# isinaltinkaya/vcfgl

Measured on AMD Instinct MI355X. Metric: site-sample GL evals/s at depth 20, 1/2/4/8 MI355X; % HBM roofline, higher is better.
Workload: dtype f64 (f32-filtered decisions, f64 fallback)

## Files before the change

### vcfgl_amd/csrc/vgl_sample.hip

```cpp
#include <stdlib.h>
#include <type_traits>

#include "vgl_common.hip.h"

#ifndef VGL_SAMPLE_SEG_TU
__global__ __launch_bounds__(256) void k_sitebase(const VglDevParams P, const VglTilePtrs T) {
    const int ls = blockIdx.x * 256 + threadIdx.x;
    if (ls >= T.n_sites) return;
    const uint64_t h = vgl_site_hash((uint64_t)(T.site0 + ls), P.site_hash_bits);
    uint64_t xb = P.x0;
#pragma unroll 1
    for (int b = 0; b < 40; ++b)
        if ((h >> b) & 1) xb = aff(P.site_pow[b], xb);
    T.site_base[ls] = xb;
    T.site_hash[ls] = h;
    if (T.tail_base) {
        uint64_t xt = VGL_TAIL_RAND48_X0;
#pragma unroll 1
        for (int b = 0; b < 40; ++b)
            if ((h >> b) & 1) xt = aff(P.site_pow[b], xt);
        T.tail_base[ls] = xt;
    }
}

template <bool ZT>
__global__ __launch_bounds__(256) void k_depth(const VglDevParams P, const VglTilePtrs T, const int chunk) {
    const int lane = threadIdx.x & 63;
    const uint32_t N = (uint32_t)P.n_samples;
    const int64_t E = (int64_t)T.n_sites * N;
    const int64_t c0 = ((int64_t)blockIdx.x * 4 + __builtin_amdgcn_readfirstlane((int)(threadIdx.x >> 6))) * chunk;
    if (c0 >= E) return;
    const int cn = (int)((E - c0 < chunk) ? (E - c0) : chunk);
    const uint32_t ls_c0 = (uint32_t)(c0 / (int64_t)N);
    const uint32_t s_c0 = (uint32_t)(c0 - (int64_t)ls_c0 * N);
    const bool big_n = N >= (uint32_t)chunk;
    auto start_of = [&](const int i, uint32_t& s_out) -> uint64_t {
        const uint32_t t = s_c0 + (uint32_t)i;
        const uint32_t add = big_n ? (uint32_t)(t >= N) : (N == 1u ? t : __umulhi(t, P.depth_magic));
        s_out = t - add * N;
        return aff(P.depth_tab[s_out], T.site_base[ls_c0 + add]);
    };

    int i = lane, next_free = 64;
    bool busy = i < cn;
    uint32_t s_i;
    uint64_t st = start_of(busy ? i : 0, s_i);
    VglPois pp = P.pois0;
    if (P.per_sample_depth) pp = P.pois[s_i];
    while (__ballot(busy)) {
        const uint64_t st1 = lcg_next(st), st2 = lcg_next(st1);
        bool neg, reject; int result;
        poisson_attempt<ZT>(pp, st1, st2, busy, P.gamma_ln_tab, P.gamma_ln_n, P.pois_zt, neg, reject, result);
        st = neg ? st1 : st2;
        const bool done = busy && !neg && !reject;
        if (done) T.dp_pre[c0 + i] = result;
        const uint64_t dm = __ballot(done);
        const int rank = (int)__builtin_amdgcn_mbcnt_hi((uint32_t)(dm >> 32), __builtin_amdgcn_mbcnt_lo((uint32_t)dm, 0u));
        const int i_n = done ? next_free + rank : i;
        next_free += __popcll(dm);
        const bool busy_n = done ? (i_n < cn) : busy;
        uint32_t s_n;
        const uint64_t st_n = start_of(busy_n ? i_n : 0, s_n);
        if (P.per_sample_depth) { const VglPois pn = P.pois[s_n]; if (done) pp = pn; }
        st = done ? st_n : st;
        i = i_n; busy = busy_n;
    }
}

#endif

template <int EQS, bool DBG, int DM, bool PREC, int LEAN, int SEG = 0>
__device__ __forceinline__ void k_sample_body(const VglDevParams& P, const VglTilePtrs& T, const int64_t wave_index) {
    constexpr bool DEFER = (LEAN >= 2);
#ifndef VGL_POOL_GROUPS
#define VGL_POOL_GROUPS 4
#endif
#ifndef VGL_POOL_ATTEMPTS
#define VGL_POOL_ATTEMPTS 2
#endif
#ifdef VGL_POOL_F64
    constexpr bool F32 = false;
#else
#ifdef VGL_PREC_F64
    constexpr bool F32 = DEFER && !PREC;
#else
    constexpr bool F32 = DEFER;
#endif
#endif
    constexpr bool P16 = F32;
    constexpr int ISZ = P16 ? 2 : 4;
    constexpr bool SLIM = (LEAN == 1 || LEAN == 2);
    constexpr bool DUMP = (LEAN == 0);
#ifdef VGL_TEST_HOOKS
    const int dbg_redo_every = P.dbg_redo_every, dbg_qs_exact = P.dbg_qs_exact;
#else
    constexpr int dbg_redo_every = 0, dbg_qs_exact = 0;
#endif
    extern __shared__ __attribute__((aligned(16))) uint8_t lds_raw[];
    const WavePos wp = wave_pos_of(P, T, wave_index);
    if (!wp.valid) return;
    const int lane = threadIdx.x & 63;
    const int N = P.n_samples;
    const int ls = wp.ls;
    const int s = wp.chunk * 64 + lane;
    const bool active = s < N;
    const size_t ev0 = (size_t)ls * N + (size_t)wp.chunk * 64;
    size_t ev = ev0 + (active ? lane : 0);
    const size_t plane = (size_t)T.n_sites * N;

    int dp = 0, a0 = 0, a1 = 0;
    int wave_total_reads = 0;
    uint64_t ad4 = 0, adf4 = 0;
    uint32_t qs0 = 0, qs1 = 0, qs2 = 0, qs3 = 0, qq0 = 0, qq1 = 0, qq2 = 0, qq3 = 0;
    uint64_t st_hap = 0, st_base = 0, st_qs = 0;
    unsigned long long c_t0 = 0, c_pois = 0, c_owner = 0, c_pool = 0, c_flush = 0, c_iter = 0, c_items = 0, c_tmp = 0;
    unsigned long long c_ntest = 0, c_gtest = 0, c_finb = 0, c_lhave = 0, c_lfin = 0, c_lhold = 0;
    if (DBG) c_t0 = clock64();
    uint64_t err_thresh = P.err_thresh;
    const bool k_strand = SLIM ? false : (LEAN == 4 ? true : (P.sample_strand != 0));
    const bool k_qsum = SLIM ? false : (LEAN == 4 ? true : (P.need_qsum != 0));
    const int k_adj = (SLIM || LEAN == 4) ? 0 : P.adjust_qs;

    const uint64_t xb = T.site_base[ls];

    if (active) {
        const VglAffine ms = P.samp_tab[s];
        const uint64_t xe = aff(ms, xb);
        st_hap = aff(P.off[1], xe);
        st_base = aff(P.off[2], xe);
        st_qs = aff(P.off[3], xe);

        int n;
        if (DM == 1) n = T.dp_pre[ev];
        else {
            uint64_t st_depth = aff(P.off[0], xe);
            VglPois pc = P.pois0;
            if (P.per_sample_depth) pc = P.pois[s];
            if (DM == 2) {
                double t = 1.0;
                int em = -1;
                uint64_t s52 = st_depth << 4;
                uint32_t k3ff = 0x3FF00000u;
                asm volatile("" : "+v"(k3ff));
                do { ++em; s52 = lcg_next52r(s52); t *= bits_1xxx_52r(s52, k3ff) - 1.0; } while (t > pc.g);
                n = em;
            } else n = poisson_draw_fast(pc, st_depth, P.gamma_ln_tab, P.gamma_ln_n);
        }
        const uint32_t g = T.gt[ev];
        a0 = g & 0xF; a1 = (g >> 4) & 0xF;
        dp = (a0 == 0xF || a1 == 0xF) ? 0 : n;
        if (dp > P.read_cap) { atomicOr(T.errflag, VGL_DEVERR_CAPACITY); dp = P.read_cap; }
#ifdef VGL_EXP_FIXED_DP
        if (EQS != 2 && dp > 0) dp = VGL_EXP_FIXED_DP;
#endif
    }

    if (DBG) c_pois = clock64() - c_t0;
    if (DBG && P.dbg_phase == 1) return;
    if (EQS == 1) {
        uint32_t lo = 0, hi = 0;
        if (lane == 0) {
            uint64_t st_site = aff(P.off[3], aff(P.samp_tab[0], xb));
            const double pe = beta_draw(P, st_site);
            if (T.site_pick_err && wp.chunk == 0) T.site_pick_err[ls] = pe;
            const uint64_t th = (uint64_t)ceil(ldexp(pe, 48));
            lo = (uint32_t)th; hi = (uint32_t)(th >> 32);
        }
        lo = __shfl(lo, 0, 64); hi = __shfl(hi, 0, 64);
        err_thresh = ((uint64_t)hi << 32) | lo;
    }

    if (EQS != 2) {
        const int q_i = P.pre_q, aq_i = P.pre_adjq;
        const uint32_t q_gl = (uint32_t)((P.adjust_qs & 1) ? aq_i : q_i);
        const uint32_t qq = (uint32_t)((P.adjust_qs & 2) ? aq_i : q_i);
        const uint32_t q2 = (uint32_t)qs_to_qssq((int)qq);
        const bool stage = P.stage_fixed != 0;
        uint64_t st_hap16 = st_hap << 16, st_base16 = st_base << 16;
        const uint64_t err_thresh16 = sample_thresh16(err_thresh);
        uint32_t* const reads_w = (uint32_t*)T.reads;
        if (SLIM) {
            const uint32_t qrep = (q_gl << 2) * 0x01010101u;
            uint32_t* const col = reads_w + ev;
            auto emit = [&](const int trip, const uint32_t bases) { if (stage) col[(size_t)trip * plane] = staged_word_of(bases, qrep); };
#ifdef VGL_FIXED_READS_V1
            const bool narrow = false;
#else
            const bool narrow = P.read_cap <= 255;
#endif
            if (narrow) {
                if (__ballot(active && dp > 0 && a0 != a1) == 0) ad4 = sample_reads_fixed<true>(st_hap16, st_base16, a0, a1, dp, err_thresh16, emit);
                else ad4 = sample_reads_fixed<false>(st_hap16, st_base16, a0, a1, dp, err_thresh16, emit);
            } else {
                if (__ballot(active && dp > 0 && a0 != a1) == 0) ad4 = sample_reads_fixed_wide<true>(st_hap16, st_base16, a0, a1, dp, err_thresh16, emit);
                else ad4 = sample_reads_fixed_wide<false>(st_hap16, st_base16, a0, a1, dp, err_thresh16, emit);
            }
        } else
        for (int r0 = 0; r0 < dp; r0 += 4) {
            uint32_t rw = 0;
#pragma unroll
            for (int j = 0; j < 4; ++j) {
                const int r = r0 + j;
                if (r < dp) {
                    bool fwd;
                    const int r_base = sample_read_base16(st_hap16, st_base16, a0, a1, err_thresh16, k_strand, fwd);
                    rw |= ((q_gl << 2) | (uint32_t)r_base) << (8 * j);
                    if (DUMP) { if (T.reads_out && r < T.reads_out_cap) T.reads_out[(size_t)r * plane + ev] = (uint8_t)((q_i << 2) | r_base); }
                    const uint64_t one = 1ULL << (16 * r_base);
                    ad4 += one;
                    if (k_strand) { if (fwd) adf4 += one; }
                }
            }
            if (stage) reads_w[(size_t)(r0 >> 2) * plane + ev] = rw;
        }
        if (P.need_qsum) {
            qs0 = qq * (uint32_t)(ad4 & 0xFFFF); qs1 = qq * (uint32_t)((ad4 >> 16) & 0xFFFF);
            qs2 = qq * (uint32_t)((ad4 >> 32) & 0xFFFF); qs3 = qq * (uint32_t)((ad4 >> 48) & 0xFFFF);
            qq0 = q2 * (uint32_t)(ad4 & 0xFFFF); qq1 = q2 * (uint32_t)((ad4 >> 16) & 0xFFFF);
            qq2 = q2 * (uint32_t)((ad4 >> 32) & 0xFFFF); qq3 = q2 * (uint32_t)((ad4 >> 48) & 0xFFFF);
        }
    } else {
        const int cap = P.pool_cap;
        uint8_t* wl = lds_raw;
        uint64_t* l_stq = (uint64_t*)wl;
        double* l_gc = (double*)(wl + 512);
        uint32_t* l_it = (uint32_t*)(wl + 576);
        uint8_t* l_pb = wl + 576 + 4 * ((size_t)cap + 2);
        uint32_t* l_ctr = l_it + cap + 1;
        const bool qfast = (LEAN >= 3) && (P.qsum_lds != 0);
        uint32_t* l_accB = (uint32_t*)(wl + ((576 + 4 * ((size_t)cap + 2) + (size_t)cap + 7) & ~(size_t)7));
        if ((uint32_t)(uintptr_t)(__attribute__((address_space(3))) uint8_t*)lds_raw != 0u) {
            if (lane == 0) atomicOr(T.errflag, VGL_DEVERR_INTERNAL);
            return;
        }

        const int incl = (int)wave_incl_scan_u32((uint32_t)dp);
        const int offs = incl - dp;
        const int total = __builtin_amdgcn_readlane(incl, 63);
        wave_total_reads = total;
        l_stq[lane] = st_qs << 4;
        uint8_t* const l_lut = wl + ((576 + 2 * ((size_t)cap + 2) + 7) & ~(size_t)7);
        uint32_t* const l_qs = (uint32_t*)(l_lut + (P.n_qs_bins != 0 ? 256 : 0));
        double* const l_gcd = (double*)((uint8_t*)l_qs + ((LEAN >= 3 && P.qsum_lds) ? 1024 : 0));
        if (F32 && PREC) { if (lane == 0) { l_gcd[0] = P.gx.a1; l_gcd[1] = P.gx.a2; l_gcd[2] = P.gy.a1; l_gcd[3] = P.gy.a2; } }
        if (P16 && P.n_qs_bins != 0) {
#pragma unroll
            for (int j = 0; j < 4; ++j) {
                const int qv = lane * 4 + j;
                int b = 0xFF;
                for (int i = 0; i < P.n_qs_bins; ++i) if (b == 0xFF && qv >= P.qs_bins[3 * i] && qv <= P.qs_bins[3 * i + 1]) b = P.qs_bins[3 * i + 2] & 0xFF;
                l_lut[qv] = (uint8_t)b;
            }
        }
        if (P16 && LEAN >= 3) { if (P.qsum_lds) { ((uint64_t*)l_qs)[2 * lane] = 0ULL; ((uint64_t*)l_qs)[2 * lane + 1] = 0ULL; } }
        if (lane == 0) {
            if (!P16) l_it[cap] = 0u;
            if (F32) {
                float* const gf = (float*)l_gc;
                gf[0] = (float)P.gx.a1; gf[1] = (float)P.gx.a2; gf[2] = (float)((((P.gx.a2 * P.gx.a2) * 0.15) * (1.0 + 1e-5) + 1e-8) * 4294967296.0); gf[3] = (float)((P.sure_margin + 3e-7) * 4294967296.0);
                gf[4] = (float)P.gy.a1; gf[5] = (float)P.gy.a2; gf[6] = (float)((((P.gy.a2 * P.gy.a2) * 0.15) * (1.0 + 1e-5) + 1e-8) * 4294967296.0); gf[7] = (float)((P.sure_margin + 3e-7) * 4294967296.0);
            } else {
            l_gc[0] = P.gx.a1; l_gc[1] = P.gx.a2; l_gc[2] = (P.gx.a2 * P.gx.a2) * 0.15; l_gc[3] = P.sure_margin;
            l_gc[4] = P.gy.a1; l_gc[5] = P.gy.a2; l_gc[6] = (P.gy.a2 * P.gy.a2) * 0.15; l_gc[7] = P.sure_margin;
            }
        }
        int rdone = 0;
        uint32_t carry_w = 0;
        uint64_t st_hap16 = st_hap << 16, st_base16 = st_base << 16;
        const uint64_t err_thresh16 = sample_thresh16(err_thresh);
        uint8_t* reads_v = T.reads;
        uint8_t* reads_out_v = DUMP ? T.reads_out : nullptr;
        int reads_out_cap_v = (DUMP && T.reads_out) ? T.reads_out_cap : 0;
        if (!DUMP) { if constexpr (SEG != 1) asm volatile("" : "+v"(reads_v)); }
        else asm volatile("" : "+v"(reads_v), "+v"(reads_out_v), "+v"(reads_out_cap_v));

        const bool homw = __ballot(active && dp > 0 && a0 != a1) == 0;
        const int nseg = (total + cap - 1) / (cap > 0 ? cap : 1);
        const int seglen = nseg > 1 ? (total + nseg - 1) / nseg : cap;
        auto run_segment = [&](auto single_tag, const int seg0) -> bool {
            constexpr bool SINGLE = decltype(single_tag)::value;
            (void)SINGLE;
            const int segT = (total - seg0 < seglen) ? (total - seg0) : seglen;
            if (DBG) c_tmp = clock64();
            int r_end = seg0 + segT - offs; r_end = r_end > dp ? dp : r_end; r_end = r_end < rdone ? rdone : r_end;
            {
                typedef __attribute__((address_space(3))) uint32_t lds_u32o;
                typedef __attribute__((address_space(3))) uint8_t lds_u8o;
                typedef __attribute__((address_space(3))) uint16_t lds_u16o;
                const uint32_t lane4 = (uint32_t)lane << 2;
                uint32_t sv = P16 ? (((uint32_t)lane << 10) | ((uint32_t)rdone << 2)) : (((uint32_t)lane << 19) | ((uint32_t)rdone << 4));
                const uint32_t sv_end = P16 ? (((uint32_t)lane << 10) | ((uint32_t)r_end << 2)) : (((uint32_t)lane << 19) | ((uint32_t)r_end << 4));
                uint32_t ka = 576u + (uint32_t)ISZ * (uint32_t)(offs + rdone - seg0);
                uint32_t pa = 576u + 4u * ((uint32_t)cap + 2u) + (uint32_t)(offs + rdone - seg0);
                auto owner_reads = [&](auto hom_tag) {
                    constexpr bool HOMW = decltype(hom_tag)::value;
                    if constexpr (SLIM) {
                        uint32_t n1 = 0;
                        const uint32_t nrd = (sv_end > sv) ? ((sv_end - sv) >> (P16 ? 2 : 4)) : 0u;
#ifdef VGL_OWNER_READS_V2
                        uint32_t hl = (uint32_t)(st_hap16 >> 12), hh = (uint32_t)(st_hap16 >> 44), bl = (uint32_t)(st_base16 >> 12), bh = (uint32_t)(st_base16 >> 44);
                        const uint32_t t_lo = (uint32_t)(err_thresh16 >> 12), t_hi = (uint32_t)(err_thresh16 >> 44);
                        while (sv < sv_end) {
                            uint32_t rb = (uint32_t)a0;
                            if (!HOMW) {
                                lcg52_step(hl, hh, hl, hh);
                                const uint32_t h = (hh >> 19) & 1u;
                                n1 += h;
                                rb = h ? (uint32_t)a1 : (uint32_t)a0;
                            }
                            lcg52_step(bl, bh, bl, bh);
                            if (__builtin_expect((bh & 0xFFFFFu) <= t_hi, 0)) {
                                if ((bh & 0xFFFFFu) < t_hi || bl < t_lo) {
                                    const uint32_t tb = rb;
                                    do { lcg52_step(bl, bh, bl, bh); rb = (bh >> 18) & 3u; } while (rb == tb);
                                    ad4 += (1ULL << (16 * rb)) - (1ULL << (16 * tb));
                                }
                            }
                            if (P16) { *(lds_u16o*)(uintptr_t)ka = (uint16_t)(sv | rb); sv += 4u; ka += 2u; }
                            else { *(lds_u32o*)(uintptr_t)ka = sv; *(lds_u8o*)(uintptr_t)pa = (uint8_t)rb; sv += 16u; ka += 4u; pa += 1u; }
                        }
                        if constexpr (SEG != 1) {
                            st_hap16 = ((((uint64_t)(hh & 0xFFFFFu)) << 32) | hl) << 12;
                            st_base16 = ((((uint64_t)(bh & 0xFFFFFu)) << 32) | bl) << 12;
                        }
#else
                        while (sv < sv_end) {
                            uint32_t rb = (uint32_t)a0;
                            if (!HOMW) {
                                st_hap16 = lcg_next16(st_hap16);
                                const uint32_t h = (uint32_t)(st_hap16 >> 63);
                                n1 += h;
                                rb = h ? (uint32_t)a1 : (uint32_t)a0;
                            }
                            st_base16 = lcg_next16(st_base16);
                            if (st_base16 < err_thresh16) {
                                const uint32_t tb = rb;
                                do { st_base16 = lcg_next16(st_base16); rb = (uint32_t)(st_base16 >> 62); } while (rb == tb);
                                ad4 += (1ULL << (16 * rb)) - (1ULL << (16 * tb));
                            }
                            if (P16) { *(lds_u16o*)(uintptr_t)ka = (uint16_t)(sv | rb); sv += 4u; ka += 2u; }
                            else { *(lds_u32o*)(uintptr_t)ka = sv; *(lds_u8o*)(uintptr_t)pa = (uint8_t)rb; sv += 16u; ka += 4u; pa += 1u; }
                        }
#endif
                        ad4 += (((uint64_t)(nrd - n1)) << (16 * (a0 & 3))) + (((uint64_t)n1) << (16 * (a1 & 3)));
                    } else if constexpr (P16) {
                        uint32_t n1 = 0, nf = 0, nf1 = 0;
                        const uint32_t nrd = (sv_end > sv) ? ((sv_end - sv) >> 2) : 0u;
                        while (sv < sv_end) {
                            uint32_t rb = (uint32_t)a0, h = 0;
                            if (!HOMW) {
                                st_hap16 = lcg_next16(st_hap16);
                                h = (uint32_t)(st_hap16 >> 63);
                                n1 += h;
                                rb = h ? (uint32_t)a1 : (uint32_t)a0;
                            }
                            const uint32_t tb = rb;
                            st_base16 = lcg_next16(st_base16);
                            const bool err = st_base16 < err_thresh16;
                            if (err) { do { st_base16 = lcg_next16(st_base16); rb = (uint32_t)(st_base16 >> 62); } while (rb == tb); }
                            uint32_t f = 1u;
                            if (k_strand) { st_base16 = lcg_next16(st_base16); f = (uint32_t)(~st_base16 >> 63); }
                            nf += f; nf1 += f & h;
                            if (err) {
                                const uint64_t d = (1ULL << (16 * rb)) - (1ULL << (16 * tb));
                                ad4 += d;
                                if (f) adf4 += d;
                            }
                            *(lds_u16o*)(uintptr_t)ka = (uint16_t)(sv | rb); sv += 4u; ka += 2u;
                        }
                        ad4 += (((uint64_t)(nrd - n1)) << (16 * (a0 & 3))) + (((uint64_t)n1) << (16 * (a1 & 3)));
                        adf4 += (((uint64_t)(nf - nf1)) << (16 * (a0 & 3))) + (((uint64_t)nf1) << (16 * (a1 & 3)));
                    } else
                    while (sv < sv_end) {
                        bool fwd;
                        const int r_base = sample_read_base16<HOMW>(st_hap16, st_base16, a0, a1, err_thresh16, k_strand, fwd);
                        const uint64_t one = 1ULL << (16 * r_base);
                        ad4 += one;
                        if (!SLIM) { if (fwd) adf4 += one; }
                        if (P16) { *(lds_u16o*)(uintptr_t)ka = (uint16_t)(sv | (uint32_t)r_base); sv += 4u; ka += 2u; }
                        else {
                            *(lds_u32o*)(uintptr_t)ka = sv;
                            *(lds_u8o*)(uintptr_t)pa = (uint8_t)((LEAN >= 3) ? (lane4 | (uint32_t)r_base) : (uint32_t)r_base);
                            sv += 16u; ka += 4u; pa += 1u;
                        }
                    }
                };
                if (homw) owner_reads(std::true_type{}); else owner_reads(std::false_type{});
            }
            if (lane == 0) {
                if (P16) ((uint16_t*)l_it)[segT] = 0; else { l_it[segT] = 0u; *l_ctr = 128u * 4u; }
            }
            __builtin_amdgcn_fence(__ATOMIC_RELEASE, "wavefront");
            __builtin_amdgcn_wave_barrier();
            __builtin_amdgcn_fence(__ATOMIC_ACQUIRE, "wavefront");

            if (DBG) { const unsigned long long c = clock64(); c_owner += c - c_tmp; c_tmp = c; c_items += segT; }
            if (DBG && P.dbg_phase == 2) return true;
            {
                typedef __attribute__((address_space(3))) uint32_t lds_u32;
                typedef __attribute__((address_space(3))) uint16_t lds_u16;
                constexpr int NGRP = F32 ? VGL_POOL_GROUPS : 1;
                const int grpQ = (segT + NGRP - 1) / NGRP;
                const int grp = (NGRP > 1) ? (lane / (64 / NGRP)) : 0, gl = (NGRP > 1) ? (lane % (64 / NGRP)) : lane;
                const int beg = grp * grpQ;
                const int endg = (beg + grpQ < segT) ? (beg + grpQ) : segT;
                const int segT4 = (NGRP > 1 || P16) ? endg * ISZ : segT * ISZ;
                int k = (beg + gl) * ISZ, kn = (beg + gl + 64 / NGRP) * ISZ;
                bool have = k < segT4;
                bool stage1 = false;
                uint64_t st = 0; double gx = 0.0; uint32_t it_m = 0;
                uint32_t sk = 0;
                if (have) {
                    if (P16) { sk = ((const uint16_t*)l_it)[beg + gl]; st = aff52(P.qs_read_tab[(sk >> 2) & 0xFFu], l_stq[sk >> 10]); }
                    else { it_m = l_it[beg + gl]; st = aff52(P.qs_read_tab[(it_m & 0xFFFFu) >> 4], l_stq[it_m >> 19]); }
                }
                if (NGRP > 1 || P16) {
                    if (gl == 0) *(lds_u32*)(uintptr_t)(544u + 4u * (uint32_t)grp) = (uint32_t)(beg + 2 * (64 / NGRP)) * (uint32_t)ISZ;
                    __builtin_amdgcn_fence(__ATOMIC_RELEASE, "wavefront");
                    __builtin_amdgcn_wave_barrier();
                    __builtin_amdgcn_fence(__ATOMIC_ACQUIRE, "wavefront");
                }
                const bool any_changed = (P.gx.changed | P.gy.changed) != 0;
                int slow_cnt = P.slow_period, slow_cnt_n = P.slow_period_n;
                uint32_t k3ff = 0x3FF00000u;
                __attribute__((address_space(3))) uint32_t* ctr_p = (NGRP > 1 || P16) ? (__attribute__((address_space(3))) uint32_t*)(uintptr_t)(544u + 4u * (uint32_t)grp)
                                                                                : (__attribute__((address_space(3))) uint32_t*)l_ctr;
                uint32_t four_v = (uint32_t)ISZ;
                asm volatile("" : "+v"(ctr_p), "+v"(four_v));
                if constexpr (F32) {
                    typedef __attribute__((address_space(3))) float lds_f32;
                    uint32_t s_lo = (uint32_t)st, s_hi = (uint32_t)(st >> 32);
                    float gxf = 0.0f;
                    double gxd = 0.0;
                    do {
                        if (DBG) { c_iter++; c_lhave += (unsigned)__popcll(__builtin_amdgcn_ballot_w64(have)); }
                        const bool full = (--slow_cnt == 0);
                        if (full) slow_cnt = P.slow_period;
                        const bool full_n = full;
                        uint32_t goff = stage1 ? 528u : 512u;
                        asm volatile("" : "+v"(goff));
                        const lds_f32* const gc = (const lds_f32*)(uintptr_t)goff;
                        const float ga1 = gc[0], ga2 = gc[1], c015s = gc[2], sure_ms = gc[3];
                        uint32_t l1, h1, l2, h2, l3, h3;
                        lcg52_step(s_lo, s_hi, l1, h1);
                        lcg52_step(l1, h1, l2, h2);
                        lcg52_step(l2, h2, l3, h3);
                        const float ufA = pool32_u(lcg52_top32(l1, h1));
                        const float svA = pool32_sv(lcg52_top32(l2, h2));
                        const float qA = pool32_q(ufA, svA);
                        const bool q_lo = qA > VGL_P32_QLO - VGL_P32_QBAND, q_hi = qA > VGL_P32_QHI + VGL_P32_QBAND;
                        bool slow_n = false;
                        const bool n_amb = have && q_lo && !q_hi;
                        bool hold = n_amb && !full_n;
                        bool redo = false;
                        if (full_n && __builtin_amdgcn_ballot_w64(n_amb)) {
                            bool und;
                            if (DBG) c_ntest++;
                            slow_n = pool32_normal_slow(svA * __builtin_amdgcn_rcpf(ufA), ufA, qA, n_amb, und);
                            redo = und || (n_amb && dbg_redo_every && (l1 >> 8) % (uint32_t)(dbg_redo_every | (dbg_redo_every == 0)) == 0u);
                        }
                        const bool accA = !(q_lo && (q_hi || slow_n));
#if VGL_POOL_ATTEMPTS == 2
                        uint32_t l4, h4, l5, h5;
                        lcg52_step(l3, h3, l4, h4);
                        lcg52_step(l4, h4, l5, h5);
                        const float ufB = pool32_u(lcg52_top32(l3, h3));
                        const float svB = pool32_sv(lcg52_top32(l4, h4));
                        const float qB = pool32_q(ufB, svB);
                        const bool rejA = have && !hold && !accA && !redo;
                        const bool useB = rejA && !(qB > VGL_P32_QLO - VGL_P32_QBAND);
                        const bool rejB = rejA && (qB > VGL_P32_QHI + VGL_P32_QBAND);
                        const float uf = useB ? ufB : ufA, sv = useB ? svB : svA;
                        const float u2f = useB ? pool32_u(lcg52_top32(l5, h5)) : ufB;
                        const bool g_try0 = (have && accA && !hold) || useB;
#else
                        const float uf = ufA, sv = svA;
                        const float u2f = pool32_u(lcg52_top32(l3, h3));
                        const bool g_try0 = have && accA && !hold;
#endif
                        asm volatile("s_waitcnt lgkmcnt(0)" : "+v"(kn));
#ifdef VGL_POOL_CLAMP_NEXT
                        const uint32_t kc = (uint32_t)(kn < segT4 ? kn : segT * ISZ);
#else
                        const uint32_t kc = P16 ? (uint32_t)kn : (uint32_t)(kn < segT4 ? kn : segT * ISZ);
#endif
                        uint32_t rd16, ow8, skn = 0;
                        if (P16) {
                            skn = *(const lds_u16*)(uintptr_t)(576u + kc);
                            asm volatile("" : "+v"(skn));
                            rd16 = (skn << 2) & 0xFF0u;
                            ow8 = (skn >> 7) & 0x1F8u;
                        } else {
                            rd16 = *(const lds_u16*)(uintptr_t)(576u + kc);
                            ow8 = *(const lds_u16*)(uintptr_t)(578u + kc);
                            asm volatile("" : "+v"(rd16), "+v"(ow8));
                        }
                        const VglAffine tab_n = *(const VglAffine*)((const uint8_t*)P.qs_read_tab + rd16);
                        const uint64_t base_n = *(__attribute__((address_space(3))) const uint64_t*)(uintptr_t)ow8;
                        const float xn = sv * __builtin_amdgcn_rcpf(uf);
                        const float w = __builtin_fmaf(ga2, xn, 1.0f);
                        const float vv = (w * w) * w;
                        const float xsq = xn * xn;
                        const float x4 = xsq * xsq;
                        const bool sure = (0x1p32f - u2f) >= __builtin_fmaf(x4, c015s, sure_ms);
                        const bool in_range = (w >= 0.5f) && (uf >= VGL_P32_UMIN);
                        redo = redo || (g_try0 && !in_range);
                        const bool g_try = g_try0 && in_range;
                        const bool g_amb = g_try && !sure;
                        hold = hold || (g_amb && !full);
                        bool slow_g = false;
                        if (full && __builtin_amdgcn_ballot_w64(g_amb)) {
                            bool und;
                            if (DBG) c_gtest++;
                            slow_g = pool32_gamma_slow(u2f, ga2 * xn, ga1, x4, g_amb, und);
                            redo = redo || und || (g_amb && dbg_redo_every && (l3 >> 8) % (uint32_t)(dbg_redo_every | (dbg_redo_every == 0)) == 1u);
                        }
                        const bool acc_g = g_try && !(g_amb && slow_g) && !hold;
#if VGL_POOL_ATTEMPTS == 2
                        {
                            const uint32_t t_lo = useB ? l5 : l3, t_hi = useB ? h5 : h3;
                            const uint32_t r_lo = rejB ? l4 : l2, r_hi = rejB ? h4 : h2;
                            s_lo = hold ? s_lo : (g_try0 ? t_lo : r_lo);
                            s_hi = hold ? s_hi : (g_try0 ? t_hi : r_hi);
                        }
#else
                        s_lo = hold ? s_lo : (g_try0 ? l3 : l2);
                        s_hi = hold ? s_hi : (g_try0 ? h3 : h2);
#endif
                        const float val = ga1 * vv;
                        const bool fin = (acc_g && stage1) || redo;
                        const float gx_prev = gxf;
                        if constexpr (PREC) {
#ifdef VGL_EXP_NO_CHAIN
                            if (false) {
#else
                            if (acc_g) {
#endif
#if VGL_POOL_ATTEMPTS == 2
                                const uint32_t ulo = useB ? l3 : l1, uhi = useB ? h3 : h1, vlo = useB ? l4 : l2, vhi = useB ? h4 : h2;
#else
                                const uint32_t ulo = l1, uhi = h1, vlo = l2, vhi = h2;
#endif
                                const double ud = bits_1xxx_52r(((uint64_t)uhi << 32) | ulo, k3ff) - 1.0;
                                const double vd = 1.7156 * (bits_1xxx_52r(((uint64_t)vhi << 32) | vlo, k3ff) - 1.5);
                                const __attribute__((address_space(3))) double* const gd = (const __attribute__((address_space(3))) double*)(uintptr_t)((uint32_t)(uintptr_t)(__attribute__((address_space(3))) uint8_t*)l_gcd + (stage1 ? 16u : 0u));
                                const double a1d = gd[0], a2d = gd[1];
                                const double xd = div_inrange(vd, ud);
                                const double wd = 1.0 + a2d * xd;
                                const double vald = a1d * (wd * wd * wd);
                                if (stage1) {
                                    if (!redo) {
                                        const size_t ei = vgl_errp_index((int)((sk >> 2) & 0xFFu), ev0 + (sk >> 10), P.read_cap);
#ifdef VGL_EXP_NO_ERRP_STORE
                                        const double epx = div_inrange(gxd, gxd + vald); if (epx > 2.0) T.errp[ei] = epx;
#else
                                        T.errp[ei] = div_inrange(gxd, gxd + vald);
#endif
                                    }
                                } else gxd = vald;
                            }
                        }
                        gxf = (acc_g && !stage1) ? val : gxf;
                        stage1 = (stage1 != acc_g) && !redo;
                        if (DBG) {
                            const uint64_t fm = __builtin_amdgcn_ballot_w64(fin);
                            c_finb += (fm != 0); c_lfin += (unsigned)__popcll(fm); c_lhold += (unsigned)__popcll(__builtin_amdgcn_ballot_w64(hold));
                        }
                        if (fin) {
                            const float pf = gx_prev * __builtin_amdgcn_rcpf(gx_prev + val);
                            if (P16) {
                                int q_i, aq_i;
                                bool ok = qs_decide_fix(P, pf, q_i, aq_i, k_adj) && !redo;
                                if (dbg_redo_every) ok = ok && ((uint32_t)(seg0 + (k >> 1)) % (uint32_t)(dbg_redo_every | (dbg_redo_every == 0))) != 2u;
                                uint32_t qv, aqv = 0;
                                if (P.n_qs_bins != 0) {
                                    const uint32_t b = l_lut[q_i < 255 ? q_i : 255];
                                    uint32_t b2 = 0;
                                    if (!SLIM) { if (k_adj) { const int a_ = aq_i < 0 ? 0 : aq_i; b2 = l_lut[a_ < 255 ? a_ : 255]; } }
                                    const bool nobin = ok && (b == 0xFFu || b2 == 0xFFu);
                                    if (__builtin_expect(__builtin_amdgcn_ballot_w64(nobin) != 0, 0)) { if (nobin) atomicOr(T.errflag, VGL_DEVERR_QSBIN); }
                                    qv = (b == 0xFFu) ? 0u : b; aqv = (b2 == 0xFFu) ? 0u : b2;
                                } else {
                                    qv = (uint32_t)((q_i > CAP_BASEQ) ? CAP_BASEQ : q_i);
                                    if (!SLIM) aqv = (uint32_t)((aq_i > CAP_BASEQ) ? CAP_BASEQ : (aq_i < 0 ? 0 : aq_i));
                                }
                                const uint32_t q_gl = SLIM ? qv : ((k_adj & 1) ? aqv : qv), q_sum = SLIM ? 0u : ((k_adj & 2) ? aqv : qv);
                                uint32_t hi6 = ok ? ((q_gl << 2) | (q_sum << 9)) : 0x100u;
                                asm volatile("" : "+v"(hi6));
                                *(lds_u16*)(uintptr_t)(576u + (uint32_t)k) = (uint16_t)(hi6 | (sk & 3u));
                                if (!SLIM) {
                                    if (qfast && k_qsum && ok)
                                        __hip_atomic_fetch_add(l_qs + ((sk >> 10) * 4u + (sk & 3u)), q_sum + ((q_sum * q_sum) << 13), __ATOMIC_RELAXED, __HIP_MEMORY_SCOPE_WAVEFRONT);
                                }
                                sk = skn;
                            } else
                            *(lds_u32*)(uintptr_t)(576u + (uint32_t)k) = redo ? 0x7FC00000u : __float_as_uint(pf);
                            aff52_step(tab_n, (uint32_t)base_n, (uint32_t)(base_n >> 32), s_lo, s_hi);
                            k = kn;
                            asm volatile("" : "+v"(k));
                            asm volatile("ds_add_rtn_u32 %0, %1, %2" : "+v"(kn) : "v"(ctr_p), "v"(four_v) : "memory");
                        }
                        have = k < segT4;
                    } while (__builtin_amdgcn_ballot_w64(have));
                } else
                do {
                    if (DBG) c_iter++;
                    const bool full = (--slow_cnt == 0);
                    if (full) slow_cnt = P.slow_period;
                    const bool full_n = (--slow_cnt_n == 0);
                    if (full_n) slow_cnt_n = P.slow_period_n;
                    uint32_t goff = stage1 ? 32u : 0u;
                    asm volatile("" : "+v"(goff));
                    const __attribute__((address_space(3))) double* gc = (const __attribute__((address_space(3))) double*)(uintptr_t)goff + 64;
                    const double ga1 = gc[0], ga2 = gc[1], ga2sq015 = gc[2], sure_margin = gc[3];
                    uint64_t st1 = lcg_next52r(st);
                    asm volatile("" : "+v"(st1));
                    const uint64_t st2 = lcg_next52r(st1);
                    const uint64_t st3 = lcg_next52r(st2);
                    const double u = bits_1xxx_52r(st1, k3ff) - 1.0;
                    const double v = 1.7156 * (bits_1xxx_52r(st2, k3ff) - 1.5);
                    const double x = u - 0.449871;
                    const double y = fabs(v) + 0.386595;
                    const double q = (x * x) + y * (0.19600 * y - 0.25472 * x);
                    const bool q_lo = q > 0.27597, q_hi = q > 0.27846;
                    bool slow_n = false;
                    const bool n_amb = have && q_lo && !q_hi;
                    bool hold = n_amb && !full_n;
                    bool redo = false;
                    if (full_n && __builtin_amdgcn_ballot_w64(n_amb)) {
                        bool und;
                        slow_n = normal_slow_test_t<DEFER>(v, u, n_amb, und);
                        if (DEFER) redo = und || (n_amb && dbg_redo_every && ((uint32_t)(st1 >> 8) % (uint32_t)(dbg_redo_every | (dbg_redo_every == 0))) == 0u);
                    }
                    const bool acc_n = !(q_lo && (q_hi || slow_n));
                    asm volatile("s_waitcnt lgkmcnt(0)" : "+v"(kn));
                    const uint32_t kc = (uint32_t)(kn < segT4 ? kn : segT4);
                    uint32_t rd16 = *(const lds_u16*)(uintptr_t)(576u + kc);
                    uint32_t ow8 = *(const lds_u16*)(uintptr_t)(578u + kc);
                    asm volatile("" : "+v"(rd16), "+v"(ow8));
                    const uint32_t m_n = PREC ? (rd16 | (ow8 << 16)) : 0u;
                    const VglAffine tab_n = *(const VglAffine*)((const uint8_t*)P.qs_read_tab + rd16);
                    const uint64_t base_n = *(__attribute__((address_space(3))) const uint64_t*)(uintptr_t)ow8;
                    const double xn = div_inrange(v, u);
                    const double w = 1.0 + ga2 * xn;
                    const bool w_pos = w > 0.0;
                    const double vv = w * w * w;
                    const double u2 = bits_1xxx_52r(st3, k3ff) - 1.0;
                    const double xsq = xn * xn;
                    const double x4 = xsq * xsq;
                    const bool sq_fail = u2 > 1.0 - 0.0331 * x4;
                    const bool sure = (1.0 - u2 >= __builtin_fma(ga2sq015, x4, sure_margin)) && (w >= 0.5);
                    const bool g_try = have && acc_n && w_pos && !hold;
                    const bool g_amb = g_try && sq_fail && !sure;
                    hold = hold || (g_amb && !full);
                    bool slow_g = false;
                    if (full && __builtin_amdgcn_ballot_w64(g_amb)) {
                        bool und;
                        slow_g = gamma_slow_test_t<DEFER>(u2, xsq, ga1, vv, ga2 * xn, g_amb, und);
                        if (DEFER) redo = redo || und || (g_amb && dbg_redo_every && ((uint32_t)(st3 >> 8) % (uint32_t)(dbg_redo_every | (dbg_redo_every == 0))) == 1u);
                    }
                    const bool acc_g = g_try && !(g_amb && slow_g) && !hold;
                    st = hold ? st : (g_try ? st3 : st2);
                    double val = ga1 * vv;
                    if (!DEFER && __builtin_expect(any_changed, 0)) {
                        asm volatile("" ::: "memory");
                        if (acc_g && (stage1 ? P.gy.changed : P.gx.changed)) {
                            double u3;
                            do { st = lcg_next52r(st); u3 = bits_1xxx_52r(st, k3ff) - 1.0; } while (u3 == 0.0);
                            val = pow(u3, 1.0 / (stage1 ? P.gy.alpha0 : P.gx.alpha0)) * ga1 * vv;
                        }
                    }
                    const bool fin = (acc_g && stage1) || redo;
                    const uint64_t st_n = tab_n.a * base_n + tab_n.c;
                    const double gx_prev = gx;
                    gx = (acc_g && !stage1) ? val : gx;
                    stage1 = (stage1 != acc_g) && !redo;
                    if (fin) {
                        *(lds_u32*)(uintptr_t)(576u + (uint32_t)k) = __float_as_uint(qs_stage_pf(gx_prev, val));
                        if (DEFER) { if (redo) *(lds_u32*)(uintptr_t)(576u + (uint32_t)k) = 0x7FC00000u; }
                        if (PREC) {
                            const size_t ei = vgl_errp_index((int)((it_m & 0xFFFFu) >> 4), ev0 + (it_m >> 19), P.read_cap);
                            T.errp[ei] = (DEFER ? div_inrange(gx_prev, gx_prev + val) : gx_prev / (gx_prev + val));
                            it_m = m_n;
                        }
                        st = st_n;
                        k = kn;
                        asm volatile("" : "+v"(k));
                        asm volatile("ds_add_rtn_u32 %0, %1, %2" : "+v"(kn) : "v"(ctr_p), "v"(four_v) : "memory");
                    }
                    have = k < segT4;
                } while (__builtin_amdgcn_ballot_w64(have));
                asm volatile("s_waitcnt lgkmcnt(0)" : "+v"(kn) : : "memory");
            }
            __builtin_amdgcn_fence(__ATOMIC_RELEASE, "wavefront");
            __builtin_amdgcn_wave_barrier();
            __builtin_amdgcn_fence(__ATOMIC_ACQUIRE, "wavefront");

            if constexpr (SEG == 1) { uint32_t l2 = (uint32_t)lane; asm volatile("" : "+v"(l2)); ev = ev0 + (active ? (size_t)l2 : 0); }
            if (DBG) { const unsigned long long c = clock64(); c_pool += c - c_tmp; c_tmp = c; }
            if (DBG && P.dbg_phase == 3) return true;
            if (!P16 && qfast && k_qsum) {
                l_stq[lane] = 0ULL;
                ((uint64_t*)l_accB)[lane] = 0ULL;
                __builtin_amdgcn_fence(__ATOMIC_RELEASE, "wavefront");
                __builtin_amdgcn_wave_barrier();
                __builtin_amdgcn_fence(__ATOMIC_ACQUIRE, "wavefront");
            }
            const int n_pass = P16 ? 0 : ((segT + 63) >> 6);
            const int dB = (qfast && !P16) ? (n_pass | 1) : 0;
            for (int jp = 0; jp < (qfast ? dB : n_pass); ++jp) {
                const int kb = qfast ? jp : 64 * jp;
                const int kstep = qfast ? dB : 1;
                const int kk = kb + lane * kstep;
                const bool inb = kk < segT;
                const float pf = __uint_as_float(l_it[inb ? kk : cap]);
                int q_i, aq_i;
                bool ok = qs_decide_pf(P, pf, q_i, aq_i, k_adj, F32 ? VGL_P32_TF_EXTRA : 0.0f) && !dbg_qs_exact;
                if (DEFER) { if (dbg_redo_every) ok = ok && ((uint32_t)(seg0 + kk) % (uint32_t)(dbg_redo_every | (dbg_redo_every == 0))) != 2u; }
                uint64_t amb = __ballot(inb && !ok);
                if (__builtin_expect(amb != 0, 0)) {
                    while (amb) {
                        const int b = __builtin_ctzll(amb);
                        amb &= amb - 1;
                        const int Kb = seg0 + kb + b * kstep;
                        if (active && Kb >= offs && Kb < offs + dp) {
                            if (DEFER) {
                                const uint32_t part = (uint32_t)wave_index & (VGL_REDO_PARTS - 1);
                                const uint32_t idx = atomicAdd(T.redo_count + VGL_REDO_STRIDE * part, 1u);
                                if (idx < T.redo_cap) T.redo_list[(size_t)part * T.redo_cap + idx] = ((unsigned long long)ev << 10) | (unsigned long long)(Kb - offs);
                                else { const size_t bit = ev * (size_t)P.read_cap + (size_t)(Kb - offs); atomicOr(&T.redo_bits[bit >> 5], 1u << (bit & 31)); }
                            } else {
                                VglAffine jr = P.qs_read_tab[Kb - offs]; jr.c >>= 4;
                                uint64_t st_x = aff(jr, l_stq[lane] >> 4);
                                const double ep = beta_draw(P, st_x);
                                int qe, aqe;
                                errprob_raw(P, ep, qe, aqe);
                                if (aqe < 0 && (P.adjust_qs & 3)) atomicOr(T.errflag, VGL_DEVERR_ADJQ);
                                l_it[kb + b * kstep] = (uint32_t)(uint16_t)qe | ((uint32_t)(uint16_t)aqe << 16);
                            }
                        }
                    }
                    if (!DEFER) {
                        __builtin_amdgcn_fence(__ATOMIC_RELEASE, "wavefront");
                        __builtin_amdgcn_wave_barrier();
                        __builtin_amdgcn_fence(__ATOMIC_ACQUIRE, "wavefront");
                        if (inb && !ok) { const uint32_t e = l_it[kk]; q_i = (int)(int16_t)(e & 0xFFFF); aq_i = (int)(int16_t)(e >> 16); }
                    } else if (inb && !ok) { q_i = 0; aq_i = SLIM ? -1 : 0; }
                }
                qs_finish(P, q_i, aq_i, T.errflag, DEFER ? (inb && ok) : inb);
                if (SLIM) { if (inb) l_pb[kk] = (uint8_t)((q_i << 2) | l_pb[kk]); }
                else if (qfast) {
                    if (inb) {
                        const uint32_t pb = l_pb[kk];
                        const uint32_t q_s = (uint32_t)((k_adj & 1) ? aq_i : q_i);
                        l_pb[kk] = (uint8_t)((q_s << 2) | (pb & 3u));
                        if (k_qsum) {
                            uint32_t* const slot = ((pb & 2u) ? l_accB : (uint32_t*)l_stq) + ((pb >> 2) * 2u + (pb & 1u));
                            __hip_atomic_fetch_add(slot, q_s + ((q_s * q_s) << 13), __ATOMIC_RELAXED, __HIP_MEMORY_SCOPE_WAVEFRONT);
                        }
                    }
                }
                else if (inb) l_it[kk] = (uint32_t)(q_i & 0xFF) | ((uint32_t)(aq_i & 0xFF) << 8);
            }
            __builtin_amdgcn_fence(__ATOMIC_RELEASE, "wavefront");
            __builtin_amdgcn_wave_barrier();
            __builtin_amdgcn_fence(__ATOMIC_ACQUIRE, "wavefront");

            uint32_t sq0 = 0, sq1 = 0, sq2 = 0, sq3 = 0, sqq0 = 0, sqq1 = 0, sqq2 = 0, sqq3 = 0;
            if (P16) {
                const uint8_t* const it8 = (const uint8_t*)l_it;
                uint8_t* reads_f = reads_v;
                if constexpr (SEG == 1) { reads_f = T.reads; asm volatile("" : "+v"(reads_f)); }
                for (int r0 = rdone & ~3; r0 < r_end; r0 += 4) {
                    uint32_t w_lo, w_hi;
                    __builtin_memcpy(&w_lo, it8 + 2 * (offs + r0 - seg0), 4);
                    __builtin_memcpy(&w_hi, it8 + 2 * (offs + r0 - seg0) + 4, 4);
                    const uint32_t w4 = __builtin_amdgcn_perm(w_hi, w_lo, 0x06040200u);
                    const int lo = rdone > r0 ? rdone - r0 : 0, hi = r_end - r0 < 4 ? r_end - r0 : 4;
                    const uint32_t mask = (0xFFFFFFFFu << (8 * lo)) & (0xFFFFFFFFu >> (8 * (4 - hi)));
                    const uint32_t rw = (w4 & mask) | ((r0 < rdone) ? carry_w : 0u);
                    ((uint32_t*)reads_f)[(size_t)(r0 >> 2) * plane + ev] = rw;
                    carry_w = rw;
                    uint32_t und4 = __builtin_amdgcn_perm(w_hi, w_lo, 0x07050301u) & mask & 0x01010101u;
                    if (__builtin_expect(und4 != 0u, 0)) {
                        while (und4) {
                            const int j = __builtin_ctz(und4) >> 3;
                            und4 &= und4 - 1;
                            const uint32_t part = (uint32_t)wave_index & (VGL_REDO_PARTS - 1);
                            const uint32_t idx = atomicAdd(T.redo_count + VGL_REDO_STRIDE * part, 1u);
                            if (idx < T.redo_cap) T.redo_list[(size_t)part * T.redo_cap + idx] = ((unsigned long long)ev << 10) | (unsigned long long)(r0 + j);
                            else { const size_t bit = ev * (size_t)P.read_cap + (size_t)(r0 + j); atomicOr(&T.redo_bits[bit >> 5], 1u << (bit & 31)); }
                        }
                    }
                    if (!SLIM) {
                        if (k_qsum && !qfast) {
#pragma unroll
                            for (int j = 0; j < 4; ++j) {
                                const uint32_t sl = ((j < 2 ? w_lo : w_hi) >> (16 * (j & 1))) & 0xFFFFu;
                                const bool mine = (r0 + j >= rdone) && (r0 + j < r_end) && !(sl & 0x100u);
                                const uint32_t qq = mine ? ((sl >> 9) & 63u) : 0u, q2 = (uint32_t)qs_to_qssq((int)qq), rb = sl & 3u;
                                sq0 += (rb == 0) ? qq : 0u; sq1 += (rb == 1) ? qq : 0u; sq2 += (rb == 2) ? qq : 0u; sq3 += (rb == 3) ? qq : 0u;
                                sqq0 += (rb == 0) ? q2 : 0u; sqq1 += (rb == 1) ? q2 : 0u; sqq2 += (rb == 2) ? q2 : 0u; sqq3 += (rb == 3) ? q2 : 0u;
                            }
                        }
                    }
                }
            } else if (SLIM || qfast) {
                for (int r0 = rdone & ~3; r0 < r_end; r0 += 4) {
                    uint32_t w4;
                    __builtin_memcpy(&w4, l_pb + (offs + r0 - seg0), 4);
                    const int lo = rdone > r0 ? rdone - r0 : 0, hi = r_end - r0 < 4 ? r_end - r0 : 4;
                    const uint32_t mask = (0xFFFFFFFFu << (8 * lo)) & (0xFFFFFFFFu >> (8 * (4 - hi)));
                    const uint32_t rw = (w4 & mask) | ((r0 < rdone) ? carry_w : 0u);
                    ((uint32_t*)reads_v)[(size_t)(r0 >> 2) * plane + ev] = rw;
                    carry_w = rw;
                }
            } else
            for (int r0 = rdone & ~3; r0 < r_end; r0 += 4) {
                uint32_t rw = (r0 < rdone) ? carry_w : 0u;
#pragma unroll
                for (int j = 0; j < 4; ++j) {
                    const int r = r0 + j;
                    if (r >= rdone && r < r_end) {
                        const int k = offs + r - seg0;
                        const int r_base = l_pb[k] & 3;
                        const uint32_t qe = l_it[k];
                        const int q_i = (int)(qe & 0xFF);
                        const int aq_i = k_adj ? (int)((qe >> 8) & 0xFF) : -1;
                        const int q_gl = (k_adj & 1) ? aq_i : q_i;
                        rw |= (uint32_t)((q_gl << 2) | r_base) << (8 * j);
                        if (DUMP) { if (r < reads_out_cap_v) reads_out_v[(size_t)r * plane + ev] = (uint8_t)((q_i << 2) | r_base); }
                        if (k_qsum) {
                            const uint32_t qq = (uint32_t)((k_adj & 2) ? aq_i : q_i);
                            const uint32_t q2 = (uint32_t)qs_to_qssq((int)qq);
                            sq0 += (r_base == 0) ? qq : 0u; sq1 += (r_base == 1) ? qq : 0u;
                            sq2 += (r_base == 2) ? qq : 0u; sq3 += (r_base == 3) ? qq : 0u;
                            sqq0 += (r_base == 0) ? q2 : 0u; sqq1 += (r_base == 1) ? q2 : 0u;
                            sqq2 += (r_base == 2) ? q2 : 0u; sqq3 += (r_base == 3) ? q2 : 0u;
                        }
                    }
                }
                ((uint32_t*)reads_v)[(size_t)(r0 >> 2) * plane + ev] = rw;
                carry_w = rw;
            }
            rdone = r_end;
            if (!SLIM) {
                if (P16 && qfast && k_qsum) {
                    const uint64_t v01 = ((const uint64_t*)l_qs)[2 * lane], v23 = ((const uint64_t*)l_qs)[2 * lane + 1];
                    sq0 = (uint32_t)v01 & 0x1FFFu; sqq0 = (uint32_t)v01 >> 13; sq1 = (uint32_t)(v01 >> 32) & 0x1FFFu; sqq1 = (uint32_t)(v01 >> 32) >> 13;
                    sq2 = (uint32_t)v23 & 0x1FFFu; sqq2 = (uint32_t)v23 >> 13; sq3 = (uint32_t)(v23 >> 32) & 0x1FFFu; sqq3 = (uint32_t)(v23 >> 32) >> 13;
                    ((uint64_t*)l_qs)[2 * lane] = 0ULL; ((uint64_t*)l_qs)[2 * lane + 1] = 0ULL;
                } else if (qfast && k_qsum) {
                    const uint64_t v01 = l_stq[lane], v23 = ((const uint64_t*)l_accB)[lane];
                    sq0 = (uint32_t)v01 & 0x1FFFu; sqq0 = (uint32_t)v01 >> 13; sq1 = (uint32_t)(v01 >> 32) & 0x1FFFu; sqq1 = (uint32_t)(v01 >> 32) >> 13;
                    sq2 = (uint32_t)v23 & 0x1FFFu; sqq2 = (uint32_t)v23 >> 13; sq3 = (uint32_t)(v23 >> 32) & 0x1FFFu; sqq3 = (uint32_t)(v23 >> 32) >> 13;
                    if (seg0 + seglen < total) {
                        __builtin_amdgcn_fence(__ATOMIC_RELEASE, "wavefront"); __builtin_amdgcn_wave_barrier();
                        if (active) l_stq[lane] = aff(P.off[3], aff(P.samp_tab[s], xb)) << 4;
                        else l_stq[lane] = 0ULL;
                    }
                }
                if (k_qsum) {
                    if (active) {
                        uint32_t* q = T.qsum + (size_t)ls * 4 * N + s;
                        if (seg0 == 0) { q[0] = sq0; q[(size_t)N] = sq1; q[(size_t)2 * N] = sq2; q[(size_t)3 * N] = sq3; }
                        else { q[0] += sq0; q[(size_t)N] += sq1; q[(size_t)2 * N] += sq2; q[(size_t)3 * N] += sq3; }
                        if (P.need_qsumsq) {
                            uint32_t* qq = T.qsumsq + (size_t)ls * 4 * N + s;
                            if (seg0 == 0) { qq[0] = sqq0; qq[(size_t)N] = sqq1; qq[(size_t)2 * N] = sqq2; qq[(size_t)3 * N] = sqq3; }
                            else { qq[0] += sqq0; qq[(size_t)N] += sqq1; qq[(size_t)2 * N] += sqq2; qq[(size_t)3 * N] += sqq3; }
                        }
                    }
// ... 309 lines not shown
```

Measured before the change: 6.208 billion.

## Run two gamma-stage attempts per pool iteration in f32 lean kernels

Adds a HALVES path for the f32 non-precise lean variants. Each loop iteration now tries the first gamma stage and then a second, fast-path-only attempt at the next stage using fresh LCG draws, so one iteration can finish a whole beta sample instead of needing two iterations. The aim is fewer loop iterations, less lane divergence and fewer waits per completed sample. The cost is more work per iteration, wasted draws when lanes hold or finish early, and higher register pressure. The shared table prefetch is factored into a lambda used by both paths.

```diff
diff --git a/vcfgl_amd/csrc/vgl_sample.hip b/vcfgl_amd/csrc/vgl_sample.hip
--- a/vcfgl_amd/csrc/vgl_sample.hip
+++ b/vcfgl_amd/csrc/vgl_sample.hip
@@ -78,6 +78,9 @@
 #ifndef VGL_POOL_ATTEMPTS
 #define VGL_POOL_ATTEMPTS 2
 #endif
+#ifndef VGL_POOL_HALVES
+#define VGL_POOL_HALVES 3
+#endif
 #ifdef VGL_POOL_F64
     constexpr bool F32 = false;
 #else
@@ -89,6 +92,7 @@
 #endif
     constexpr bool P16 = F32;
     constexpr int ISZ = P16 ? 2 : 4;
+    constexpr bool HALVES = F32 && !PREC && ((VGL_POOL_HALVES >> (LEAN == 2 ? 0 : (LEAN == 4 ? 1 : 2))) & 1) != 0;
     constexpr bool SLIM = (LEAN == 1 || LEAN == 2);
     constexpr bool DUMP = (LEAN == 0);
 #ifdef VGL_TEST_HOOKS
@@ -441,6 +445,109 @@
                         asm volatile("" : "+v"(goff));
                         const lds_f32* const gc = (const lds_f32*)(uintptr_t)goff;
                         const float ga1 = gc[0], ga2 = gc[1], c015s = gc[2], sure_ms = gc[3];
+                        uint32_t skn = 0;
+                        VglAffine tab_n;
+                        uint64_t base_n;
+                        auto prefetch = [&]() {
+                            asm volatile("s_waitcnt lgkmcnt(0)" : "+v"(kn));
+#ifdef VGL_POOL_CLAMP_NEXT
+                            const uint32_t kc = (uint32_t)(kn < segT4 ? kn : segT * ISZ);
+#else
+                            const uint32_t kc = P16 ? (uint32_t)kn : (uint32_t)(kn < segT4 ? kn : segT * ISZ);
+#endif
+                            uint32_t rd16, ow8;
+                            if (P16) {
+                                skn = *(const lds_u16*)(uintptr_t)(576u + kc);
+                                asm volatile("" : "+v"(skn));
+                                rd16 = (skn << 2) & 0xFF0u;
+                                ow8 = (skn >> 7) & 0x1F8u;
+                            } else {
+                                rd16 = *(const lds_u16*)(uintptr_t)(576u + kc);
+                                ow8 = *(const lds_u16*)(uintptr_t)(578u + kc);
+                                asm volatile("" : "+v"(rd16), "+v"(ow8));
+                            }
+                            tab_n = *(const VglAffine*)((const uint8_t*)P.qs_read_tab + rd16);
+                            base_n = *(__attribute__((address_space(3))) const uint64_t*)(uintptr_t)ow8;
+                        };
+                        bool hold, redo, fin;
+                        float fx, fy;
+                        if constexpr (HALVES) {
+                            uint32_t l1, h1, l2, h2, l3, h3;
+                            lcg52_step(s_lo, s_hi, l1, h1);
+                            lcg52_step(l1, h1, l2, h2);
+                            lcg52_step(l2, h2, l3, h3);
+                            const float ufA = pool32_u(lcg52_top32(l1, h1));
+                            const float svA = pool32_sv(lcg52_top32(l2, h2));
+                            const float u2A = pool32_u(lcg52_top32(l3, h3));
+                            const float qA = pool32_q(ufA, svA);
+                            const bool q_lo = qA > VGL_P32_QLO - VGL_P32_QBAND, q_hi = qA > VGL_P32_QHI + VGL_P32_QBAND;
+                            const bool n_amb = have && q_lo && !q_hi;
+                            bool slow_n = false;
+                            hold = n_amb && !full;
+                            redo = false;
+                            const float xnA = svA * __builtin_amdgcn_rcpf(ufA);
+                            if (full && __builtin_amdgcn_ballot_w64(n_amb)) {
+                                bool und;
+                                if (DBG) c_ntest++;
+                                slow_n = pool32_normal_slow(xnA, ufA, qA, n_amb, und);
+                                redo = und || (n_amb && dbg_redo_every && (l1 >> 8) % (uint32_t)(dbg_redo_every | (dbg_redo_every == 0)) == 0u);
+                            }
+                            const bool g_try0 = have && !hold && !(q_lo && (q_hi || slow_n));
+                            prefetch();
+                            const float wA = __builtin_fmaf(ga2, xnA, 1.0f);
+                            const float xsqA = xnA * xnA;
+                            const float x4A = xsqA * xsqA;
+                            const bool sureA = (0x1p32f - u2A) >= __builtin_fmaf(x4A, c015s, sure_ms);
+                            const bool in_rangeA = (wA >= 0.5f) && (ufA >= VGL_P32_UMIN);
+                            redo = redo || (g_try0 && !in_rangeA);
+                            const bool g_try = g_try0 && in_rangeA;
+                            const bool g_amb = g_try && !sureA;
+                            hold = hold || (g_amb && !full);
+                            bool slow_g = false;
+                            if (full && __builtin_amdgcn_ballot_w64(g_amb)) {
+                                bool und;
+                                if (DBG) c_gtest++;
+                                slow_g = pool32_gamma_slow(u2A, ga2 * xnA, ga1, x4A, g_amb, und);
+                                redo = redo || und || (g_amb && dbg_redo_every && (l3 >> 8) % (uint32_t)(dbg_redo_every | (dbg_redo_every == 0)) == 1u);
+                            }
+                            const bool acc1 = g_try && !(g_amb && slow_g) && !hold;
+                            const float val1 = ga1 * ((wA * wA) * wA);
+                            const bool fin1 = (acc1 && stage1) || redo;
+                            s_lo = hold ? s_lo : (g_try0 ? l3 : l2);
+                            s_hi = hold ? s_hi : (g_try0 ? h3 : h2);
+                            gxf = (acc1 && !stage1) ? val1 : gxf;
+                            stage1 = (stage1 != acc1) && !redo;
+                            uint32_t goff2 = stage1 ? 528u : 512u;
+                            asm volatile("" : "+v"(goff2));
+                            const lds_f32* const gc2 = (const lds_f32*)(uintptr_t)goff2;
+                            const float gb1 = gc2[0], gb2 = gc2[1], c015s2 = gc2[2], sure_ms2 = gc2[3];
+                            uint32_t m1, n1, m2, n2, m3, n3;
+                            lcg52_step(s_lo, s_hi, m1, n1);
+                            lcg52_step(m1, n1, m2, n2);
+                            lcg52_step(m2, n2, m3, n3);
+                            const float ufB = pool32_u(lcg52_top32(m1, n1));
+                            const float svB = pool32_sv(lcg52_top32(m2, n2));
+                            const float u2B = pool32_u(lcg52_top32(m3, n3));
+                            const float qB = pool32_q(ufB, svB);
+                            const bool run2 = have && !hold && !fin1;
+                            const bool rej2 = run2 && (qB > VGL_P32_QHI + VGL_P32_QBAND);
+                            const float xnB = svB * __builtin_amdgcn_rcpf(ufB);
+                            const float wB = __builtin_fmaf(gb2, xnB, 1.0f);
+                            const float xsqB = xnB * xnB;
+                            const float x4B = xsqB * xsqB;
+                            const bool sureB = (0x1p32f - u2B) >= __builtin_fmaf(x4B, c015s2, sure_ms2);
+                            const bool in_rangeB = (wB >= 0.5f) && (ufB >= VGL_P32_UMIN);
+                            const bool acc2 = run2 && !(qB > VGL_P32_QLO - VGL_P32_QBAND) && in_rangeB && sureB;
+                            const float val2 = gb1 * ((wB * wB) * wB);
+                            s_lo = acc2 ? m3 : (rej2 ? m2 : s_lo);
+                            s_hi = acc2 ? n3 : (rej2 ? n2 : s_hi);
+                            const bool fin2 = acc2 && stage1;
+                            fin = fin1 || fin2;
+                            fx = gxf;
+                            fy = fin2 ? val2 : val1;
+                            gxf = (acc2 && !stage1) ? val2 : gxf;
+                            stage1 = stage1 != acc2;
+                        } else {
                         uint32_t l1, h1, l2, h2, l3, h3;
                         lcg52_step(s_lo, s_hi, l1, h1);
                         lcg52_step(l1, h1, l2, h2);
@@ -451,8 +558,8 @@
                         const bool q_lo = qA > VGL_P32_QLO - VGL_P32_QBAND, q_hi = qA > VGL_P32_QHI + VGL_P32_QBAND;
                         bool slow_n = false;
                         const bool n_amb = have && q_lo && !q_hi;
-                        bool hold = n_amb && !full_n;
-                        bool redo = false;
+                        hold = n_amb && !full_n;
+                        redo = false;
                         if (full_n && __builtin_amdgcn_ballot_w64(n_amb)) {
                             bool und;
                             if (DBG) c_ntest++;
@@ -478,25 +585,7 @@
                         const float u2f = pool32_u(lcg52_top32(l3, h3));
                         const bool g_try0 = have && accA && !hold;
 #endif
-                        asm volatile("s_waitcnt lgkmcnt(0)" : "+v"(kn));
-#ifdef VGL_POOL_CLAMP_NEXT
-                        const uint32_t kc = (uint32_t)(kn < segT4 ? kn : segT * ISZ);
-#else
-                        const uint32_t kc = P16 ? (uint32_t)kn : (uint32_t)(kn < segT4 ? kn : segT * ISZ);
-#endif
-                        uint32_t rd16, ow8, skn = 0;
-                        if (P16) {
-                            skn = *(const lds_u16*)(uintptr_t)(576u + kc);
-                            asm volatile("" : "+v"(skn));
-                            rd16 = (skn << 2) & 0xFF0u;
-                            ow8 = (skn >> 7) & 0x1F8u;
-                        } else {
-                            rd16 = *(const lds_u16*)(uintptr_t)(576u + kc);
-                            ow8 = *(const lds_u16*)(uintptr_t)(578u + kc);
-                            asm volatile("" : "+v"(rd16), "+v"(ow8));
-                        }
-                        const VglAffine tab_n = *(const VglAffine*)((const uint8_t*)P.qs_read_tab + rd16);
-                        const uint64_t base_n = *(__attribute__((address_space(3))) const uint64_t*)(uintptr_t)ow8;
+                        prefetch();
                         const float xn = sv * __builtin_amdgcn_rcpf(uf);
                         const float w = __builtin_fmaf(ga2, xn, 1.0f);
                         const float vv = (w * w) * w;
@@ -527,9 +616,8 @@
                         s_lo = hold ? s_lo : (g_try0 ? l3 : l2);
                         s_hi = hold ? s_hi : (g_try0 ? h3 : h2);
 #endif
-                        const float val = ga1 * vv;
-                        const bool fin = (acc_g && stage1) || redo;
-                        const float gx_prev = gxf;
+                        fin = (acc_g && stage1) || redo;
+                        fx = gxf; fy = ga1 * vv;
                         if constexpr (PREC) {
 #ifdef VGL_EXP_NO_CHAIN
                             if (false) {
@@ -560,14 +648,15 @@
                                 } else gxd = vald;
                             }
                         }
-                        gxf = (acc_g && !stage1) ? val : gxf;
+                        gxf = (acc_g && !stage1) ? fy : gxf;
                         stage1 = (stage1 != acc_g) && !redo;
+                        }
                         if (DBG) {
                             const uint64_t fm = __builtin_amdgcn_ballot_w64(fin);
                             c_finb += (fm != 0); c_lfin += (unsigned)__popcll(fm); c_lhold += (unsigned)__popcll(__builtin_amdgcn_ballot_w64(hold));
                         }
                         if (fin) {
-                            const float pf = gx_prev * __builtin_amdgcn_rcpf(gx_prev + val);
+                            const float pf = fx * __builtin_amdgcn_rcpf(fx + fy);
                             if (P16) {
                                 int q_i, aq_i;
                                 bool ok = qs_decide_fix(P, pf, q_i, aq_i, k_adj) && !redo;
```

After: 6.571 billion (median of 6 runs). +5.9%, better.
